# idcrook/tweeker_raytracer

Hardware: AMD Instinct MI355X
Metric: Msamples/s (paths x spp x res / s), Cornell box 1920x1080 (higher is better)
Workload: dtype f32; 1 GPU; C2: Cornell box (scene_rtigo3_cornell_box.txt: Lambert + GGX wall + mirror + glass spheres, 64,096 triangles, 8 instances), 1920x1080, 2534 spp progressive (1 spp per step), pathLengths 2 10, light 1, miss 0; launch_width=1920, batch_depth=64, parallelism=single GPU

## Files before the change

tweeker_raytracer_amd/csrc/device_api.hip:

```cpp
#include "device_types.h"
#include "bvh_build.h"
#include "error_state.h"

#include <algorithm>
#include <chrono>
#include <cmath>
#include <cstdlib>
#include <cstring>
#include <string>
#include <vector>

static thread_local std::string g_lastError;

int twkSetError(int code, const std::string& message)
{
  g_lastError = message;
  return code;
}

namespace twk {
void launchTrace(const LaunchParams& p, int depth, bool count, bool primary, int gridBlocks, hipStream_t stream);
void launchTraceQuery(const LaunchParams& p, const float* rays, unsigned int numRays, int anyHit, float* tBetaGamma, int* ids, int gridBlocks, hipStream_t stream);
void launchGenerate(const LaunchParams& p, hipStream_t stream);
void launchShade(const LaunchParams& p, int depth, bool primary, int gridBlocks, hipStream_t stream);
// ... 73 lines not shown
  bool built = false;
  bool twoLevel = true;
  int  flattenMaxTriangles = TWK_FLATTEN_TRIANGLES, flattenMaxReferences = TWK_FLATTEN_REFERENCES;
  int  maxInstanceMaterial = -1, maxInstanceLight = -1;
  TwkBuildInfo buildInfo;

  float* d_camera = nullptr;
  DevLight* d_lights = nullptr;
  DevMaterial* d_materials = nullptr; int materialCapacity = 0;
  float* d_attributes = nullptr; unsigned int* d_indices = nullptr;
  BvhNode* d_nodes = nullptr; BvhNode* d_wideNodes = nullptr ; float4* d_wideQ = nullptr; float4* d_triangles = nullptr; float4* d_shadeTriangles = nullptr; DevInstance* d_instances = nullptr;
  bool directSmallLeaves = true;  bool costedCuts = true;  bool fusedPrimary = true;  bool tileEntries = true;  bool wideRoot = true;  int wideRoot1 = 0, wideRoot2 = TWK_BVH_SENTINEL; size_t wideNodesTotal = 0;
  int4* d_tileEntries = nullptr; size_t tileEntriesCapacity = 0; TileEntriesKey tileEntriesKey = {}; uint64_t buildSerial = 0;
  float4* d_topNodes = nullptr; float4* d_topNodes7 = nullptr; bool topCache = true; int traceWavesForced = 0 ;
  float4* d_texels[3] = {nullptr, nullptr, nullptr};
  float* d_envCDF_U = nullptr; float* d_envCDF_V = nullptr;
  int tlasRoot = 0;
  size_t totalNodes = 0, totalTriangles = 0;

  int allocatedPixels = 0;
  void* d_streamBlock = nullptr;
  float4* d_outputInternal = nullptr;
  float4* d_outputExternal = nullptr; size_t outputExternalBytes = 0;
  bool outputFrame = false;
  unsigned int* d_counters = nullptr;
  unsigned long long* d_stats = nullptr;
  unsigned int* h_dropped = nullptr; unsigned int* d_dropped = nullptr;
  int* d_spill = nullptr; size_t spillLanes = 0;
  bool packedQueue = true;
  int shadeSort = 1;
  float4* d_firstHit = nullptr; int* d_firstHitInstance = nullptr;
  bool aovEnabled = false; int shaderVariant = TWK_SHADERS_RTIGO3;
  bool nextEventEstimation = true, debugExceptions = false;
  bool timeView = false; float* d_pathTime = nullptr; int timePaths = 0;
  float4* d_pathAlbedo = nullptr; float4* d_pathNormal = nullptr; int aovPaths = 0;
  float4* d_aovAlbedo = nullptr; float4* d_aovNormal = nullptr; int aovPixels = 0;
  bool captureFirstHits = false;
  bool statsEnabled = false;
  bool profileEnabled = false;
  std::vector<TimedLaunch> timed; size_t timedUsed = 0;
  float profileMs[TWK_KERNEL_COUNT] = {0, 0, 0, 0, 0};
  int   profileLaunches[TWK_KERNEL_COUNT] = {0, 0, 0, 0, 0};
  int   batchMax = 64;
  size_t streamBudgetBytes = 0;
  unsigned int pendingFirst = 0;
  int   pendingCount = 0;
  int   allocatedPaths = 0;

  hipStream_t laneStream[TWK_MAX_LANES] = {nullptr, nullptr, nullptr, nullptr};
  hipEvent_t  laneDone[TWK_MAX_LANES] = {nullptr, nullptr, nullptr, nullptr};
  hipEvent_t  laneFork = nullptr;
  int   lanesForced = 0;
  int   laneTraceWaves = 0;

  std::vector<std::vector<char>> hostScene;

  LaunchParams params;
  BvhBuilder builder;
};

static int flushPending(TwkDevice dev);

static int activate(TwkDevice dev, const char* where, bool flush = true)
{
  if (!dev) return twkSetError(TWK_ERROR_INVALID_VALUE, std::string(where) + ": NULL device handle");
  HIP_TRY(hipSetDevice(dev->ordinal));
  if (flush && dev->pendingCount > 0) return flushPending(dev);
  return TWK_SUCCESS;
}

template<typename T> static void freeDevice(T*& p) { if (p) { (void) hipFree(p); p = nullptr; } }

template<typename T> struct ScopedDeviceBuffer
{
  T* ptr = nullptr;
  ~ScopedDeviceBuffer() { if (ptr) (void) hipFree(ptr); }
  hipError_t allocate(size_t count) { return hipMalloc(&ptr, count * sizeof(T)); }
};

static void invertAffine(const float m[12], float inv[12])
{
  const double a00 = m[0], a01 = m[1], a02 = m[2],  t0 = m[3];
  const double a10 = m[4], a11 = m[5], a12 = m[6],  t1 = m[7];
  const double a20 = m[8], a21 = m[9], a22 = m[10], t2 = m[11];
  const double c00 = a11 * a22 - a12 * a21;
  const double c01 = a12 * a20 - a10 * a22;
  const double c02 = a10 * a21 - a11 * a20;
  const double det = a00 * c00 + a01 * c01 + a02 * c02;
  const double r = 1.0 / det;
  const double i00 = c00 * r, i01 = (a02 * a21 - a01 * a22) * r, i02 = (a01 * a12 - a02 * a11) * r;
  const double i10 = c01 * r, i11 = (a00 * a22 - a02 * a20) * r, i12 = (a02 * a10 - a00 * a12) * r;
  const double i20 = c02 * r, i21 = (a01 * a20 - a00 * a21) * r, i22 = (a00 * a11 - a01 * a10) * r;
  inv[0] = (float) i00; inv[1] = (float) i01; inv[2]  = (float) i02; inv[3]  = (float) -(i00 * t0 + i01 * t1 + i02 * t2);
  inv[4] = (float) i10; inv[5] = (float) i11; inv[6]  = (float) i12; inv[7]  = (float) -(i10 * t0 + i11 * t1 + i12 * t2);
  inv[8] = (float) i20; inv[9] = (float) i21; inv[10] = (float) i22; inv[11] = (float) -(i20 * t0 + i21 * t1 + i22 * t2);
}

static DevMaterial convertMaterial(const TwkMaterialGUI& g)
{
  DevMaterial m;
  memset(&m, 0, sizeof(m));
  m.textureAlbedo = g.useAlbedoTexture ? (TWK_TEXTURE_ALBEDO + 1) : 0;
  m.textureCutout = g.useCutoutTexture ? (TWK_TEXTURE_CUTOUT + 1) : 0;
  m.roughness[0] = g.roughness[0]; m.roughness[1] = g.roughness[1];
  m.indexBSDF = g.indexBSDF;
  m.albedo[0] = g.albedo[0]; m.albedo[1] = g.albedo[1]; m.albedo[2] = g.albedo[2];
// ... 18 lines not shown
}

static void refreshParams(TwkDevice dev)
{
  LaunchParams& p = dev->params;
  p.nodes = dev->d_nodes; p.wideQ = dev->d_wideQ; p.triangles = dev->d_triangles; p.shadeTriangles = dev->d_shadeTriangles; p.instances = dev->d_instances;
  p.attributes = dev->d_attributes; p.indices = dev->d_indices;
  p.materials = dev->d_materials; p.lights = dev->d_lights; p.camera = dev->d_camera;
  p.tlasRoot = dev->tlasRoot;
  p.topNodes = dev->d_topNodes; p.topNodes7 = dev->d_topNodes7;
  p.topRoot = dev->topCache ? (TWK_NODE_CACHED | 0) : dev->wideRoot1;
  p.topRoot2 = (dev->wideRoot2 == TWK_BVH_SENTINEL) ? TWK_BVH_SENTINEL : (dev->topCache ? (TWK_NODE_CACHED | 1) : dev->wideRoot2);
  p.twoLevel = dev->twoLevel ? 1 : 0;
  p.numInstances = (int) dev->instances.size();
  p.numLights = (int) dev->lights.size();
  p.numMaterials = (int) dev->materials.size();
  p.miss = dev->miss;
  p.hasCutout = 0; p.hasAlbedoTexture = 0;
  for (const DevMaterial& m : dev->materials) { if (m.textureCutout != 0) p.hasCutout = 1; if (m.textureAlbedo != 0) p.hasAlbedoTexture = 1; }
  p.traceWaves = (!dev->twoLevel && (!p.hasCutout || TWK_TRACE_CUTOUT_SEVEN) && dev->totalNodes <= (size_t) TWK_TRACE_WAVES7_MAX_NODES) ? TWK_TRACE_WAVES7 : (p.hasCutout ? (dev->twoLevel ? TWK_TRACE_WAVES_CUTOUT_OTHER : TWK_TRACE_WAVES) : TWK_TRACE_WAVES);
  if (dev->traceWavesForced == TWK_TRACE_WAVES || (dev->traceWavesForced == TWK_TRACE_WAVES7 && !dev->twoLevel)) p.traceWaves = dev->traceWavesForced;
  p.envCDF_U = dev->d_envCDF_U; p.envCDF_V = dev->d_envCDF_V;
  for (int k = 0; k < 2; ++k)
  {
    p.resolution[k]  = dev->state.resolution[k];
    p.tileSize[k]    = dev->state.tileSize[k];
    p.tileShift[k]   = calculateShift(dev->state.tileSize[k]);
    p.pathLengths[k] = dev->state.pathLengths[k];
  }
  p.deviceCount = dev->count; p.deviceIndex = dev->index; p.distribution = dev->state.distribution;
  p.launchWidth = dev->launchWidth;
  p.lensShader  = dev->state.lensShader;
  p.sceneEpsilon = dev->state.epsilonFactor * SCENE_EPSILON_SCALE;
  p.envRotation  = dev->state.envRotation;
  p.numPixels = dev->launchWidth * dev->state.resolution[1];
  p.batchCount = 1;
  p.numPaths = p.numPixels;
  p.queueStride = TWK_QUEUE_STRIDE(p.numPaths);
  p.pathBase = 0;
  p.output = dev->d_outputExternal ? dev->d_outputExternal : dev->d_outputInternal;
  p.outputFrame = (dev->d_outputExternal && dev->outputFrame) ? 1 : 0;
  p.counters = dev->d_counters;
  p.stats = dev->statsEnabled ? dev->d_stats : (dev->timeView ? dev->d_stats + TWK_STATS_WORDS / 2 : nullptr);
  p.pathTime = dev->timeView ? dev->d_pathTime : nullptr; p.clockScale = dev->state.clockFactor * 1.0e-9f;
  p.shaderVariant = dev->shaderVariant; p.shadeSort = dev->shadeSort;
  p.nextEventEstimation = dev->nextEventEstimation ? 1 : 0; p.debugExceptions = dev->debugExceptions ? 1 : 0;
  p.pathAlbedo = dev->aovEnabled ? dev->d_pathAlbedo : nullptr; p.pathNormal = dev->aovEnabled ? dev->d_pathNormal : nullptr;
  p.aovAlbedo  = dev->aovEnabled ? dev->d_aovAlbedo : nullptr;  p.aovNormal  = dev->aovEnabled ? dev->d_aovNormal : nullptr;
  p.firstHit = dev->captureFirstHits ? dev->d_firstHit : nullptr;
  p.firstHitInstance = dev->captureFirstHits ? dev->d_firstHitInstance : nullptr;
  p.traceStackSpill = dev->d_spill;
  p.droppedPushes = dev->d_dropped;
  p.packedQueue = 0;
}

static int traceGridBlocks(TwkDevice dev) { return dev->numCUs * TWK_TRACE_WAVES7; }

static int ensureStreams(TwkDevice dev, int samples = 1)
{
  const size_t wantPixels = (size_t) dev->launchWidth * (size_t) dev->state.resolution[1];
  const size_t wantPaths  = wantPixels * (size_t) (samples > 1 ? samples : 1);
  if (wantPaths >= ((size_t) 1 << 31))
    return twkSetError(TWK_ERROR_OUT_OF_MEMORY, "a pass of " + std::to_string(wantPaths) + " paths exceeds the 2^31 path indices of a wavefront pass");
  const int numPixels = (int) wantPixels;
  const int numPaths  = (int) wantPaths;
  if (numPixels > dev->allocatedPixels || dev->d_outputInternal == nullptr)
  {
    freeDevice(dev->d_outputInternal);
    freeDevice(dev->d_firstHit); freeDevice(dev->d_firstHitInstance);
    const size_t n = (size_t) numPixels;
    HIP_TRY(hipMalloc(&dev->d_outputInternal, n * sizeof(float4)));
    HIP_TRY(hipMemsetAsync(dev->d_outputInternal, 0, n * sizeof(float4), dev->stream));
    HIP_TRY(hipMalloc(&dev->d_firstHit, n * sizeof(float4)));
    HIP_TRY(hipMalloc(&dev->d_firstHitInstance, n * sizeof(int)));
    dev->allocatedPixels = numPixels;
  }
  if (numPaths > dev->allocatedPaths || dev->d_streamBlock == nullptr)
  {
    freeDevice(dev->d_streamBlock);
    const size_t n = (size_t) numPaths;
    const size_t bytes = (n + TWK_STREAM_PAD) * (15 * sizeof(float4) + 2 * sizeof(uint2) + 6 * sizeof(unsigned int)) + 4096;
    if (dev->streamBudgetBytes != 0 && n * (15 * sizeof(float4) + 2 * sizeof(uint2) + 6 * sizeof(unsigned int)) > dev->streamBudgetBytes)
      return twkSetError(TWK_ERROR_OUT_OF_MEMORY, "path streams of " + std::to_string(bytes >> 20) + " MiB exceed TWK_STREAM_BUDGET_MB");
    HIP_TRY(hipMalloc(&dev->d_streamBlock, bytes));
    dev->allocatedPaths = numPaths;
  }
  if (dev->timeView && dev->allocatedPaths > dev->timePaths)
  {
    freeDevice(dev->d_pathTime); dev->timePaths = 0;
    HIP_TRY(hipMalloc(&dev->d_pathTime, (size_t) dev->allocatedPaths * sizeof(float)));
    dev->timePaths = dev->allocatedPaths;
  }
  if (dev->aovEnabled)
  {
    if (dev->allocatedPaths > dev->aovPaths)
    {
      freeDevice(dev->d_pathAlbedo); freeDevice(dev->d_pathNormal); dev->aovPaths = 0;
      HIP_TRY(hipMalloc(&dev->d_pathAlbedo, (size_t) dev->allocatedPaths * sizeof(float4)));
      HIP_TRY(hipMalloc(&dev->d_pathNormal, (size_t) dev->allocatedPaths * sizeof(float4)));
      dev->aovPaths = dev->allocatedPaths;
    }
    if (dev->allocatedPixels > dev->aovPixels)
    {
      freeDevice(dev->d_aovAlbedo); freeDevice(dev->d_aovNormal); dev->aovPixels = 0;
      const size_t bytes = (size_t) dev->allocatedPixels * sizeof(float4);
      HIP_TRY(hipMalloc(&dev->d_aovAlbedo, bytes));
// ... 319 lines not shown
{
  if (!count) return twkSetError(TWK_ERROR_INVALID_VALUE, "twk_device_count: NULL argument");
  *count = 0;
  int n = 0;
  const hipError_t e = hipGetDeviceCount(&n);
  if (e != hipSuccess) return twkSetError(TWK_ERROR_NO_DEVICE, std::string("hipGetDeviceCount failed: ") + hipGetErrorString(e));
  *count = n;
  return TWK_SUCCESS;
}
TWK_CATCH("twk_device_count")

int twk_device_create(TwkDevice* out, int ordinal, int index, int count, int miss)
try
{
  if (!out) return twkSetError(TWK_ERROR_INVALID_VALUE, "twk_device_create: NULL out pointer");
  *out = nullptr;
  if (count < 1 || index < 0 || index >= count) return twkSetError(TWK_ERROR_INVALID_VALUE, "twk_device_create: need 0 <= index < count");
  int n = 0;
  const hipError_t e = hipGetDeviceCount(&n);
  if (e != hipSuccess || n <= 0)
    return twkSetError(TWK_ERROR_NO_DEVICE, std::string("twk_device_create: no HIP device available (") + ((e != hipSuccess) ? hipGetErrorString(e) : "device count 0") + "); this library has no CPU path");
  if (ordinal < 0 || ordinal >= n) return twkSetError(TWK_ERROR_INVALID_VALUE, "twk_device_create: device ordinal out of range");

  TwkDevice_t* dev = new TwkDevice_t();
  dev->ordinal = ordinal; dev->index = index; dev->count = count; dev->miss = miss;
  memset(&dev->params, 0, sizeof(dev->params));
  memset(&dev->state, 0, sizeof(dev->state));
  dev->state.resolution[0] = dev->state.resolution[1] = 1;
  dev->state.tileSize[0] = dev->state.tileSize[1] = 8;
  dev->state.pathLengths[0] = 2; dev->state.pathLengths[1] = 5;
  dev->state.epsilonFactor = 500.0f;
  dev->state.clockFactor = 1000.0f;

  hipError_t err = hipSetDevice(ordinal);
  if (err == hipSuccess) err = hipStreamCreateWithFlags(&dev->stream, hipStreamNonBlocking);
  hipDeviceProp_t prop;
  if (err == hipSuccess) err = hipGetDeviceProperties(&prop, ordinal);
  if (err != hipSuccess)
  {
    delete dev;
    return twkSetError(TWK_ERROR_NO_DEVICE, std::string("twk_device_create: ") + hipGetErrorString(err));
  }
  dev->numCUs = prop.multiProcessorCount > 0 ? prop.multiProcessorCount : 256;
  if (const char* e = getenv("TWK_PASS_LANES")) dev->lanesForced = std::max(0, std::min(TWK_MAX_LANES, atoi(e)));
  if (const char* e = getenv("TWK_LANE_TRACE_WAVES")) dev->laneTraceWaves = std::max(0, atoi(e));
  if (const char* e = getenv("TWK_TOP_CACHE")) dev->topCache = (atoi(e) != 0);
  if (const char* e = getenv("TWK_DIRECT_SMALL_LEAVES")) dev->directSmallLeaves = (atoi(e) != 0);
  if (const char* e = getenv("TWK_COSTED_CUTS")) dev->costedCuts = (atoi(e) != 0);
  if (const char* e = getenv("TWK_FUSED_PRIMARY")) dev->fusedPrimary = (atoi(e) != 0);
  if (const char* e = getenv("TWK_TILE_ENTRIES")) dev->tileEntries = (atoi(e) != 0);
  if (const char* e = getenv("TWK_WIDE_ROOT")) dev->wideRoot = (atoi(e) != 0);
  if (const char* e = getenv("TWK_PACKED_QUEUE")) dev->packedQueue = (atoi(e) != 0);
  if (const char* e = getenv("TWK_SHADE_SORT")) dev->shadeSort = atoi(e);
  if (const char* e = getenv("TWK_TRACE_WAVES_RUNTIME")) dev->traceWavesForced = atoi(e);
  if (const char* e = getenv("TWK_BUILD_QUALITY")) dev->builder.setQuality(atoi(e));
  memset(&dev->buildInfo, 0, sizeof(dev->buildInfo));
  if (const char* e = getenv("TWK_STREAM_BUDGET_MB")) { const long long mb = atoll(e); dev->streamBudgetBytes = (mb > 0) ? (size_t) mb << 20 : 0; }
  if (const char* e = getenv("TWK_BATCH")) { const int b = atoi(e); dev->batchMax = (b < 1) ? 1 : ((b > 64) ? 64 : b); }
  *out = dev;
  return TWK_SUCCESS;
}
TWK_CATCH("twk_device_create")

int twk_device_destroy(TwkDevice dev)
try
{
  if (!dev) return TWK_SUCCESS;
  dev->pendingCount = 0;
  (void) hipSetDevice(dev->ordinal);
  if (dev->stream) (void) hipStreamSynchronize(dev->stream);
  for (TimedLaunch& t : dev->timed) { (void) hipEventDestroy(t.start); (void) hipEventDestroy(t.stop); }
  freeDevice(dev->d_camera); freeDevice(dev->d_lights); freeDevice(dev->d_materials);
  freeDevice(dev->d_attributes); freeDevice(dev->d_indices);
  freeDevice(dev->d_nodes); freeDevice(dev->d_wideNodes); freeDevice(dev->d_wideQ); freeDevice(dev->d_triangles); freeDevice(dev->d_shadeTriangles); freeDevice(dev->d_instances);
  for (int k = 0; k < 3; ++k) freeDevice(dev->d_texels[k]);
  freeDevice(dev->d_envCDF_U); freeDevice(dev->d_envCDF_V); freeDevice(dev->d_topNodes); freeDevice(dev->d_topNodes7); freeDevice(dev->d_tileEntries);
  freeDevice(dev->d_streamBlock); freeDevice(dev->d_outputInternal);
  freeDevice(dev->d_counters); freeDevice(dev->d_stats); freeDevice(dev->d_spill); freeDevice(dev->d_pathTime);
  if (dev->h_dropped) { (void) hipHostFree(dev->h_dropped); dev->h_dropped = nullptr; dev->d_dropped = nullptr; }
  freeDevice(dev->d_firstHit); freeDevice(dev->d_firstHitInstance);
  freeDevice(dev->d_pathAlbedo); freeDevice(dev->d_pathNormal); freeDevice(dev->d_aovAlbedo); freeDevice(dev->d_aovNormal);
  dev->builder.release();
  for (int k = 1; k < TWK_MAX_LANES; ++k)
  {
    if (dev->laneStream[k]) (void) hipStreamDestroy(dev->laneStream[k]);
    if (dev->laneDone[k]) (void) hipEventDestroy(dev->laneDone[k]);
  }
  if (dev->laneFork) (void) hipEventDestroy(dev->laneFork);
  if (dev->stream) (void) hipStreamDestroy(dev->stream);
  delete dev;
  return TWK_SUCCESS;
}
TWK_CATCH("twk_device_destroy")

int twk_set_state(TwkDevice dev, const TwkDeviceState* s)
try
{
  int rc = activate(dev, "twk_set_state"); if (rc) return rc;
  if (!s) return twkSetError(TWK_ERROR_INVALID_VALUE, "twk_set_state: NULL state");
  if (s->resolution[0] < 1 || s->resolution[1] < 1) return twkSetError(TWK_ERROR_INVALID_VALUE, "twk_set_state: resolution must be >= 1");
  if (s->tileSize[0] < 1 || s->tileSize[1] < 1 || (s->tileSize[0] & (s->tileSize[0] - 1)) || (s->tileSize[1] & (s->tileSize[1] - 1)))
    return twkSetError(TWK_ERROR_INVALID_VALUE, "twk_set_state: tileSize must be a power of two");
  if (s->pathLengths[1] < 0 || s->pathLengths[1] > TWK_MAX_DEPTH) return twkSetError(TWK_ERROR_INVALID_VALUE, "twk_set_state: pathLengths.y must be in [0, 64]");
  if (s->lensShader < 0 || s->lensShader > 2) return twkSetError(TWK_ERROR_INVALID_VALUE, "twk_set_state: lensShader must be 0..2");
  HIP_TRY(hipStreamSynchronize(dev->stream));
  dev->state = *s;
// ... 966 lines not shown
```

tweeker_raytracer_amd/csrc/device_types.h:

```cpp
#pragma once
#include "device_math.h"
#include "../../include/tweeker_hip.h"

namespace twk {

static const float RT_DEFAULT_MAX      = 1.e27f;
static const float SCENE_EPSILON_SCALE = 1.0e-7f;
static const float DENOMINATOR_EPSILON = 1.0e-6f;

#define TWK_MATERIAL_STACK_EMPTY (-1)
#define TWK_MATERIAL_STACK_FIRST 0
#define TWK_MATERIAL_STACK_LAST  3
#define TWK_MATERIAL_STACK_SIZE  4
#define TWK_FLAG_HIT          0x00000001u
#define TWK_FLAG_SHADOW       0x00000002u
#define TWK_FLAG_DIFFUSE      0x00000004u
#define TWK_FLAG_LIGHT        0x00000008u
#define TWK_FLAG_FRONTFACE    0x00000010u
#define TWK_FLAG_THINWALLED   0x00000020u
#define TWK_FLAG_TRANSMISSION 0x00000100u
#define TWK_FLAG_VOLUME       0x00001000u
#define TWK_FLAG_ALBEDO       0x10000000u
#define TWK_FLAG_TERMINATE    0x80000000u
#define TWK_FLAG_CLEAR_MASK   (TWK_FLAG_DIFFUSE | TWK_FLAG_ALBEDO)
// ... 96 lines not shown
  unsigned int envWidth, envHeight;
  float envIntegral, envRotation;

  int   resolution[2];
  int   tileSize[2];
  int   tileShift[2];
  int   pathLengths[2];
  int   deviceCount, deviceIndex, distribution;
  int   launchWidth;
  int   lensShader;
  unsigned int iterationIndex;
  float sceneEpsilon;

  float4* rayOrg[2];
  float4* rayDir[2];
  unsigned int* rayPixel[2];
  float4* hitRecord;
  int*    hitInstance;
  float4* shadowOrg;
  float4* shadowDir;
  unsigned int* shadowPixel;
  float4* shadowPending;
  float4* rayThroughput[2];
  uint2*  raySeedFlags[2];
  float4* pathRadiance;
  float4* volumeStack;
  float4* pathAlbedo;
  float4* pathNormal;
  float*  pathTime;
  float   clockScale;
  float4* aovAlbedo;
  float4* aovNormal;
  int     shaderVariant;
  int     shadeSort;
  int     nextEventEstimation;
  int     debugExceptions;
  int     outputFrame;
  float4* output;
  unsigned int* counters;
  unsigned long long* stats;
  float4* firstHit;
  int*    firstHitInstance;
  int*    traceStackSpill;
  unsigned int* overflowSlots;
  int     numPixels;
  int     numPaths;
  int     batchCount;
  int     pathBase;
  const int4* tileEntries;
  int     tilesX;
  int     packedQueue;
  unsigned int queueStride;
  unsigned int* droppedPushes;
};

#ifndef TWK_QUEUE_SEGMENTS
#define TWK_QUEUE_SEGMENTS 4
#endif
#ifndef TWK_COUNTER_SEGMENT_STRIDE
#define TWK_COUNTER_SEGMENT_STRIDE 64
#endif
#define TWK_COUNTERS_PER_DEPTH (2 * TWK_QUEUE_SEGMENTS * TWK_COUNTER_SEGMENT_STRIDE + 2)
#define TWK_COUNTER_CLOSEST  0
#define TWK_COUNTER_SHADOW   (TWK_QUEUE_SEGMENTS * TWK_COUNTER_SEGMENT_STRIDE)
#define TWK_COUNTER_TICKET   (2 * TWK_QUEUE_SEGMENTS * TWK_COUNTER_SEGMENT_STRIDE)
#define TWK_COUNTER_OVERFLOW (2 * TWK_QUEUE_SEGMENTS * TWK_COUNTER_SEGMENT_STRIDE + 1)
#define TWK_QUEUE_STRIDE(numPaths) ((((unsigned int) (numPaths) / TWK_QUEUE_SEGMENTS + 255u) & ~255u) + 512u)

struct QueueSegments { unsigned int first[TWK_QUEUE_SEGMENTS]; unsigned int total; };

TWK_HD QueueSegments queueSegments(const unsigned int* counts)
{
  QueueSegments s; unsigned int sum = 0u;
  for (int k = 0; k < TWK_QUEUE_SEGMENTS; ++k) { s.first[k] = sum; sum += counts[k * TWK_COUNTER_SEGMENT_STRIDE]; }
  s.total = sum;
  return s;
}
TWK_HD QueueSegments noSegments() { QueueSegments s; for (int k = 0; k < TWK_QUEUE_SEGMENTS; ++k) s.first[k] = 0u; s.total = 0u; return s; }
TWK_HD unsigned int physicalSlot(const QueueSegments& s, unsigned int stride, unsigned int v)
{
  unsigned int k = 0u, f = 0u;
  for (int j = 1; j < TWK_QUEUE_SEGMENTS; ++j) { const bool in = v >= s.first[j]; k += in ? 1u : 0u; f = in ? s.first[j] : f; }
  return k * stride + (v - f);
}
#define TWK_MAX_DEPTH 64

#ifndef TWK_TRACE_STACK_LDS
#define TWK_TRACE_STACK_LDS   20
#endif
#ifndef TWK_TRACE_WAVES
#define TWK_TRACE_WAVES 6
#endif
#ifndef TWK_TRACE_CUTOUT_SEVEN
#define TWK_TRACE_CUTOUT_SEVEN 1
#endif
#ifndef TWK_TRACE_WAVES_CUTOUT_OTHER
#define TWK_TRACE_WAVES_CUTOUT_OTHER 5
#endif
#ifndef TWK_TRACE_WAVES_PRIMARY
#define TWK_TRACE_WAVES_PRIMARY TWK_TRACE_WAVES
#endif
#ifndef TWK_TRACE_WAVES_PRIMARY_TWO_LEVEL
#define TWK_TRACE_WAVES_PRIMARY_TWO_LEVEL 5
#endif
#define TWK_TRACE_WAVES7      7
#define TWK_TRACE_STACK_LDS7  19
#define TWK_TOP_NODES7        32
#ifndef TWK_TRACE_WAVES7_MAX_NODES
#define TWK_TRACE_WAVES7_MAX_NODES 1000000
#endif
#ifndef TWK_ENTRY_TILE
#define TWK_ENTRY_TILE 8
#endif
#define TWK_ENTRY_REFS 7
#ifndef TWK_PRIMARY_SIX
#define TWK_PRIMARY_SIX 1
#endif
#define TWK_TRACE_STACK_SPILL 72
#define TWK_TRACE_BLOCK       256
#define TWK_SHADE_BLOCKS_PER_CU 128
#ifndef TWK_SHADE_BLOCK
#define TWK_SHADE_BLOCK       256
#endif
#ifndef TWK_LANES2_MAX_PATHS
#define TWK_LANES2_MAX_PATHS 21000000
#endif
#ifndef TWK_TRACE_SMALL_CHUNK
#define TWK_TRACE_SMALL_CHUNK 64
#endif
#ifndef TWK_TRACE_CHUNK
#define TWK_TRACE_CHUNK       512
#endif

}
```

tweeker_raytracer_amd/csrc/trace_persistent.h:

```cpp
#pragma once
#include "trace_device.h"
#include "shade_device.h"

namespace twk {

TWK_D bool cutoutIgnoresCandidate(const LaunchParams& p, const TraceResult& res, bool isShadow, int q, unsigned int record, bool primary = false)
{
  const DevInstance& inst = p.instances[res.instance];
  const DevMaterial& material = p.materials[inst.material];
  if (material.textureCutout == 0) return false;
  const float4* sv = p.shadeTriangles + TWK_SHADE_RECORD * (size_t) res.triangleSlot;
  const float4 s5 = sv[5], s6 = sv[6], s7 = sv[7];
  const float alpha = 1.0f - res.beta - res.gamma;
  const V3 texcoord = v3(s5.y, s5.z, s5.w) * alpha + v3(s6.x, s6.y, s6.z) * res.beta + v3(s6.w, s7.x, s7.y) * res.gamma;
  const float opacity = intensity(v3(tex2D(p.textures[1], texcoord.x, texcoord.y)));
  if (!(opacity < 1.0f)) return false;
  float draw;
  if (isShadow)
  {
    float4 pend = p.shadowPending[record];
    unsigned int seed = __float_as_uint(pend.w);
    draw = rng(seed);
    pend.w = __uint_as_float(seed);
    p.shadowPending[record] = pend;
  }
  else
  {
    uint2 sf = p.raySeedFlags[q][record];
    draw = rng(sf.x);
    p.raySeedFlags[q][record] = sf;
  }
  if (!(opacity <= draw)) return false;
  if (isShadow) p.shadowOrg[record].w = res.t; else if (!primary) p.rayOrg[q][record].w = res.t;
  return true;
}

#ifndef TWK_TRACE_REFILL
#define TWK_TRACE_REFILL 52
#endif
#ifndef TWK_TRACE_REFILL_PRIMARY
#define TWK_TRACE_REFILL_PRIMARY 32
#endif
#ifndef TWK_TRACE_TAIL_DEN
#define TWK_TRACE_TAIL_DEN 2
#endif
#ifndef TWK_TRACE_TAIL_MIN
#define TWK_TRACE_TAIL_MIN 2u
#endif
#ifndef TWK_TRACE_NODE_NUM
#define TWK_TRACE_NODE_NUM 1
#endif
#ifndef TWK_TRACE_NODE_DEN
#define TWK_TRACE_NODE_DEN 2
#endif

template<bool COUNT, bool CUTOUT, bool TWO_LEVEL, bool W7, bool PRIMARY>
__global__ void __launch_bounds__(TWK_TRACE_BLOCK, W7 ? TWK_TRACE_WAVES7 : (CUTOUT ? ((PRIMARY || TWO_LEVEL) ? TWK_TRACE_WAVES_CUTOUT_OTHER : TWK_TRACE_WAVES) : ((PRIMARY && TWO_LEVEL) ? TWK_TRACE_WAVES_PRIMARY_TWO_LEVEL : (PRIMARY ? TWK_TRACE_WAVES_PRIMARY : TWK_TRACE_WAVES))))
traceKernel(LaunchParams p, int depth)
{
  constexpr int STACK_LDS = W7 ? TWK_TRACE_STACK_LDS7 : TWK_TRACE_STACK_LDS;
  constexpr int TOP_NODES = W7 ? TWK_TOP_NODES7 : TWK_TOP_NODES;
  constexpr int STACK_ROWS = STACK_LDS + 1;
  __shared__ int stackStorage[STACK_ROWS * TWK_TRACE_BLOCK];
  __shared__ float4 topCache[TOP_NODES * TWK_TOP_STRIDE];
  int* ldsStack = stackStorage + threadIdx.x;
  const int stride = TWK_TRACE_BLOCK;
  {
    const float4* topSource = W7 ? p.topNodes7 : p.topNodes;
    for (int i = threadIdx.x; i < TOP_NODES * 4; i += TWK_TRACE_BLOCK) topCache[(i >> 2) * TWK_TOP_STRIDE + (i & 3)] = topSource[i];
  }
  __syncthreads();

  const QueueSegments closestSegments = queueSegments(&p.counters[depth * TWK_COUNTERS_PER_DEPTH + TWK_COUNTER_CLOSEST]);
  const QueueSegments shadowSegments  = (depth > 0) ? queueSegments(&p.counters[(depth - 1) * TWK_COUNTERS_PER_DEPTH + TWK_COUNTER_SHADOW]) : noSegments();
  const unsigned int numClosest = closestSegments.total, numShadow = shadowSegments.total;
  const unsigned int total = numClosest + numShadow;
#define TWK_RECORD(slot_) (((slot_) < numClosest) ? (PRIMARY ? (slot_) : physicalSlot(closestSegments, p.queueStride, (slot_))) : physicalSlot(shadowSegments, p.queueStride, (slot_) - numClosest))

  const int q = depth & 1;
  const bool packed = !CUTOUT && !PRIMARY && p.packedQueue != 0 && depth > 0;
  const unsigned int lane = threadIdx.x & 63u;
  const unsigned long long laneBelow = (1ull << lane) - 1ull;

  unsigned int nodeCount = 0, triCount = 0, instCount = 0, closestCount = 0, shadowCount = 0, maxSteps = 0, cachedCount = 0;
  unsigned int nodeWaveSteps = 0, triWaveSteps = 0, leafWaveSteps = 0;
#define TWK_WAVE_STEP(counter) if (COUNT) { if (lane == (unsigned int) (__ffsll((long long) __ballot(true)) - 1)) ++(counter); }
  unsigned long long phaseCycles[5] = {0ull, 0ull, 0ull, 0ull, 0ull};
  unsigned long long phaseMark = COUNT ? __builtin_readcyclecounter() : 0ull;
  const unsigned long long kernelStart = phaseMark;
#define TWK_PHASE_END(k) if (COUNT) { const unsigned long long now_ = __builtin_readcyclecounter(); phaseCycles[k] += now_ - phaseMark; phaseMark = now_; }

  const unsigned int numWaves = gridDim.x * (TWK_TRACE_BLOCK / 64);
  const unsigned int waveId   = blockIdx.x * (TWK_TRACE_BLOCK / 64) + (threadIdx.x >> 6);
  unsigned int ticketSize = TWK_TRACE_CHUNK;
  const bool longQueue = total >= numWaves * ticketSize * TWK_TRACE_TAIL_MIN;
#if TWK_TRACE_SMALL_CHUNK
  if (!longQueue) ticketSize = TWK_TRACE_SMALL_CHUNK;
#else
  if (total < numWaves * ticketSize) ticketSize = min((unsigned int) TWK_TRACE_CHUNK, max(16u, ((total + numWaves - 1u) / numWaves + 15u) & ~15u));
#endif
  unsigned int nextChunk = waveId * ticketSize;
  if (nextChunk >= total) return;
  unsigned int poolBase = 0u, poolCount = 0u;
#if TWK_TRACE_TAIL_DEN
  unsigned int* ticket = &p.counters[depth * TWK_COUNTERS_PER_DEPTH + TWK_COUNTER_TICKET];
  const unsigned int staticEnd = longQueue ? ((total - total / TWK_TRACE_TAIL_DEN) / (numWaves * ticketSize)) * (numWaves * ticketSize) : total;
#else
  const unsigned int staticEnd = total;
#endif
  bool exhausted = false;

  enum : unsigned int
  {
    ST_HAS_RAY    = 1u,
    ST_ANY_HIT    = 2u,
    ST_DONE       = 4u,
    ST_SHADOW     = 8u,
    ST_RETRACE    = 16u,
    ST_OVERFLOWED = 32u,
    ST_CLOCKED    = 64u
  };
  unsigned int state = 0u;
  unsigned int slot = 0;
  V3 org = v3(0.0f), dir = v3(0.0f);
  float tmin = 0.0f;
  TraceResult res; res.t = 0.0f; res.beta = 0.0f; res.gamma = 0.0f; res.instance = -1; res.primitive = -1; res.triangleSlot = -1;
  TraceRay ray; ray.o = v3(0.0f); ray.d = v3(0.0f); ray.id = v3(0.0f);
  WoopConstants woop; woop.perm = 0u; woop.Sx = 0.0f; woop.Sy = 0.0f; woop.Sz = 0.0f;
  int currentInstance = -1, sp = 0, node = TWK_BVH_SENTINEL;
  unsigned int guard = 0;
  unsigned int rayClock = 0;

  for (;;)
  {
    if (state & ST_DONE)
    {
      const unsigned int rayCycles = COUNT ? ((state & ST_CLOCKED) ? rayClock : (unsigned int) __builtin_readcyclecounter() - rayClock) : 0u;
      state &= ~(ST_DONE | ST_CLOCKED);
      const bool isShadow = (state & ST_SHADOW) != 0u;
      if (state & ST_RETRACE)
      {
        state = (state & ~ST_RETRACE) | ST_OVERFLOWED;
        const unsigned int k = atomicAdd(&p.counters[depth * TWK_COUNTERS_PER_DEPTH + TWK_COUNTER_OVERFLOW], 1u);
        p.overflowSlots[k] = slot;
        if (PRIMARY && CUTOUT) p.hitRecord[slot] = make_float4(tmin, 0.0f, 0.0f, 0.0f);
      }
      if (COUNT) maxSteps = max(maxSteps, guard);
      const bool ignoredCandidate = CUTOUT && !(state & ST_OVERFLOWED) && res.instance >= 0 &&
                                    cutoutIgnoresCandidate(p, res, isShadow, q, TWK_RECORD(slot), PRIMARY);
      if (ignoredCandidate)
      {
        tmin = res.t;
        float4 o, d;
        if (PRIMARY)
        {
          const PrimaryRay pr = primaryRay(p, slot);
          o = make_float4(pr.origin.x, pr.origin.y, pr.origin.z, 0.0f);
          d = make_float4(pr.direction.x, pr.direction.y, pr.direction.z, RT_DEFAULT_MAX);
        }
        else
        {
          const unsigned int record = TWK_RECORD(slot);
          o = isShadow ? p.shadowOrg[record] : p.rayOrg[q][record];
          d = isShadow ? p.shadowDir[record] : p.rayDir[q][record];
        }
        org = v3(o); dir = v3(d);
        res.t = d.w; res.beta = 0.0f; res.gamma = 0.0f; res.instance = -1; res.primitive = -1; res.triangleSlot = -1;
        setupRay(ray, org, dir);
        woopSetup(dir, woop);
        if (COUNT) rayClock = (unsigned int) __builtin_readcyclecounter() - rayCycles;
        currentInstance = -1; sp = 0; node = p.topRoot; guard = 0;
        if (p.topRoot2 != TWK_BVH_SENTINEL) { ldsStack[0] = p.topRoot2; sp = 1; }
        state |= ST_HAS_RAY;
      }
      else if (state & ST_OVERFLOWED) { state &= ~ST_OVERFLOWED; }
      else if (!isShadow)
      {
        p.hitRecord[slot]   = make_float4(res.t, res.beta, res.gamma, __int_as_float(res.triangleSlot));
        p.hitInstance[slot] = res.instance;
        if (COUNT) ++closestCount;
        if (COUNT && p.pathTime != nullptr) atomicAdd(&p.pathTime[PRIMARY ? slot : (packed ? (__float_as_uint(p.rayOrg[q][TWK_RECORD(slot)].w) & TWK_PACKED_PIXEL_MASK) : p.rayPixel[q][TWK_RECORD(slot)])], float(rayCycles));
        if (p.firstHit != nullptr && depth == 0)
        {
          const unsigned int pixel = PRIMARY ? slot : p.rayPixel[q][TWK_RECORD(slot)];
          p.firstHit[pixel] = make_float4(res.t, res.beta, res.gamma, __int_as_float(res.primitive));
          p.firstHitInstance[pixel] = res.instance;
        }
      }
// ... 41 lines not shown
            slot = poolBase + rank;
            float4 o, d;
            int4 entryA = make_int4(0, 0, 0, 0), entryB = make_int4(0, 0, 0, 0);
            if (PRIMARY)
            {
              const PrimaryRay pr = primaryRay(p, slot);
              o = make_float4(pr.origin.x, pr.origin.y, pr.origin.z, p.sceneEpsilon);
              d = make_float4(pr.direction.x, pr.direction.y, pr.direction.z, pr.active ? RT_DEFAULT_MAX : -1.0f);
              state = ST_HAS_RAY;
              if (CUTOUT) p.raySeedFlags[0][slot] = make_uint2(pr.seed, 0u);
              if (p.tileEntries != nullptr)
              {
                const unsigned int launchIndex = (slot + (unsigned int) p.pathBase) % (unsigned int) p.numPixels;
                const unsigned int lx = launchIndex % (unsigned int) p.launchWidth, ly = launchIndex / (unsigned int) p.launchWidth;
                const int4* tile = p.tileEntries + 2 * ((size_t) (ly / TWK_ENTRY_TILE) * (unsigned int) p.tilesX + lx / TWK_ENTRY_TILE);
                entryA = tile[0]; entryB = tile[1];
              }
            }
            else if (slot < numClosest)
            {
              const unsigned int record = physicalSlot(closestSegments, p.queueStride, slot);
              o = p.rayOrg[q][record]; d = p.rayDir[q][record]; state = ST_HAS_RAY;
              if (packed) { o.w = p.sceneEpsilon; d.w = RT_DEFAULT_MAX; }
            }
            else
            {
              const unsigned int record = physicalSlot(shadowSegments, p.queueStride, slot - numClosest);
              o = p.shadowOrg[record]; d = p.shadowDir[record]; state = ST_HAS_RAY | ST_SHADOW | (CUTOUT ? 0u : ST_ANY_HIT);
            }
            org = v3(o); dir = v3(d); tmin = o.w;
            res.t = d.w; res.beta = 0.0f; res.gamma = 0.0f; res.instance = -1; res.primitive = -1; res.triangleSlot = -1;
            setupRay(ray, org, dir);
            woopSetup(dir, woop);
            currentInstance = -1; sp = 0; guard = 0;
            node = p.topRoot;
            if (p.topRoot2 != TWK_BVH_SENTINEL) { ldsStack[0] = p.topRoot2; sp = 1; }
            if (COUNT) rayClock = (unsigned int) __builtin_readcyclecounter();
            if (PRIMARY && entryA.x > 0)
            {
              sp = 0;
              node = entryA.y;
              const int count = entryA.x;
              if (count > 6) { ldsStack[sp * stride] = entryB.w; ++sp; }
              if (count > 5) { ldsStack[sp * stride] = entryB.z; ++sp; }
              if (count > 4) { ldsStack[sp * stride] = entryB.y; ++sp; }
              if (count > 3) { ldsStack[sp * stride] = entryB.x; ++sp; }
              if (count > 2) { ldsStack[sp * stride] = entryA.w; ++sp; }
              if (count > 1) { ldsStack[sp * stride] = entryA.z; ++sp; }
            }
          }
          poolBase += take; poolCount -= take;
        }
      }
      if (__ballot((state & ST_HAS_RAY) != 0u) == 0ull)
      {
        if (exhausted) break;
        continue;
      }
    }
    TWK_PHASE_END(0)
    for (;;)
    {
      const int roundActive = __popcll(__ballot((state & ST_HAS_RAY) != 0u));
      while ((unsigned int) node < (unsigned int) TWK_BVH_SENTINEL)
      {
        {
          float4 n0, n1, n2, n3;
          if (node & TWK_NODE_CACHED)
          {
            const float4* w = topCache + (node & 0xff) * TWK_TOP_STRIDE;
            if (COUNT) ++cachedCount;
            n0 = w[0]; n1 = w[1]; n2 = w[2]; n3 = w[3];
          }
          else
          {
            const float4* w = p.wideQ + 4 * (size_t) node;
            n0 = w[0]; n1 = w[1]; n2 = w[2]; n3 = w[3];
          }
          ++guard;
          if (COUNT) ++nodeCount;
          TWK_WAVE_STEP(nodeWaveSteps)
          int r0 = __float_as_int(n3.x), r1 = __float_as_int(n3.y), r2 = __float_as_int(n3.z), r3 = __float_as_int(n3.w);
          asm volatile("" : "+v"(r0), "+v"(r1), "+v"(r2), "+v"(r3));
          const float ax = n0.w * ray.id.x, ay = n1.x * ray.id.y, az = n1.y * ray.id.z;
          const float bx = __builtin_fmaf(n0.x, ray.id.x, -ray.ood.x), by = __builtin_fmaf(n0.y, ray.id.y, -ray.ood.y), bz = __builtin_fmaf(n0.z, ray.id.z, -ray.ood.z);
          const bool negX = ray.id.x < 0.0f, negY = ray.id.y < 0.0f, negZ = ray.id.z < 0.0f;
          const unsigned int qlx = __float_as_uint(n1.z), qly = __float_as_uint(n1.w), qlz = __float_as_uint(n2.x);
          const unsigned int qhx = __float_as_uint(n2.y), qhy = __float_as_uint(n2.z), qhz = __float_as_uint(n2.w);
          const unsigned int qnx = negX ? qhx : qlx, qfx = negX ? qlx : qhx;
          const unsigned int qny = negY ? qhy : qly, qfy = negY ? qly : qhy;
          const unsigned int qnz = negZ ? qhz : qlz, qfz = negZ ? qlz : qhz;
          float t0, t1, t2, t3;
  #define TWK_Q(word, k) ((float) (((word) >> (8 * (k))) & 0xffu))
  #define TWK_SLAB(k, tk) slabTestGrid(ax, ay, az, bx, by, bz, TWK_Q(qnx, k), TWK_Q(qny, k), TWK_Q(qnz, k), TWK_Q(qfx, k), TWK_Q(qfy, k), TWK_Q(qfz, k), tmin, res.t, tk)
          const bool h0 = TWK_SLAB(0, t0);
          const bool h1 = TWK_SLAB(1, t1);
          const bool h2 = TWK_SLAB(2, t2);
          const bool h3 = TWK_SLAB(3, t3);
  #undef TWK_SLAB
  #undef TWK_Q
          const float inf = __uint_as_float(0x7f800000u);
          t0 = h0 ? t0 : inf; t1 = h1 ? t1 : inf; t2 = h2 ? t2 : inf; t3 = h3 ? t3 : inf;
  #define TWK_CE(ta, ra, tb, rb) { const bool sw = (tb) < (ta); const float tl = sw ? (tb) : (ta); (tb) = sw ? (ta) : (tb); (ta) = tl; const int rl = sw ? (rb) : (ra); (rb) = sw ? (ra) : (rb); (ra) = rl; }
          TWK_CE(t0, r0, t1, r1) TWK_CE(t2, r2, t3, r3) TWK_CE(t0, r0, t2, r2) TWK_CE(t1, r1, t3, r3) TWK_CE(t1, r1, t2, r2)
  #undef TWK_CE
          const int hits = (int) h0 + (int) h1 + (int) h2 + (int) h3;
// ... 26 lines not shown
        TWK_WAVE_STEP(leafWaveSteps)
        if (TWO_LEVEL && node == TWK_BVH_SENTINEL)
        {
          sp -= 4;
          woop.perm = (unsigned int) ldsStack[sp * stride];
          woop.Sx = __int_as_float(ldsStack[(sp + 1) * stride]);
          woop.Sy = __int_as_float(ldsStack[(sp + 2) * stride]);
          woop.Sz = __int_as_float(ldsStack[(sp + 3) * stride]);
          setupRay(ray, org, dir);
          currentInstance = -1;
          pop = 1u;
        }
        else
        {
          const int payload = ~node;
          if (TWO_LEVEL && currentInstance < 0 && !(payload & TWK_LEAF_WORLD))
          {
            const float4* rec = reinterpret_cast<const float4*>(p.instances + payload);
            const float4 r0 = rec[0], r1 = rec[1], r2 = rec[2], r3 = rec[3];
            if (COUNT) ++instCount;
            if (sp + 5 > STACK_LDS) state = (state & ~ST_HAS_RAY) | ST_DONE | ST_RETRACE;
            else
            {
              ldsStack[sp * stride] = (int) woop.perm;
              ldsStack[(sp + 1) * stride] = __float_as_int(woop.Sx);
              ldsStack[(sp + 2) * stride] = __float_as_int(woop.Sy);
              ldsStack[(sp + 3) * stride] = __float_as_int(woop.Sz);
              ldsStack[(sp + 4) * stride] = TWK_BVH_SENTINEL;
              sp += 5;
              float m[12];
              m[0] = r0.x; m[1] = r0.y; m[2] = r0.z; m[3] = r0.w;
              m[4] = r1.x; m[5] = r1.y; m[6] = r1.z; m[7] = r1.w;
              m[8] = r2.x; m[9] = r2.y; m[10] = r2.z; m[11] = r2.w;
              const V3 objOrg = transformPoint(m, org);
              const V3 objDir = transformVector(m, dir);
              woopSetup(objDir, woop);
              setupRay(ray, objOrg, objDir);
              currentInstance = payload;
              node = __float_as_int(r3.x);
            }
          }
          else
          {
            triFirst = payload & 0x0fffffff; triLast = triFirst + ((payload >> 28) & 3);
            pop = 1u;
          }
        }

      }

      TWK_PHASE_END(2)
#define TWK_MERGE_HIT(hit_, t_, beta_, gamma_, inst_, prim_, ts_)                                                              \
      {                                                                                                                        \
        const bool closer = (hit_) & (((t_) < res.t) |                                                                         \
                                      (((t_) == res.t) & (res.instance >= 0) &                                                 \
                                       (((inst_) < res.instance) | (((inst_) == res.instance) & ((prim_) < res.primitive))))); \
        res.t = closer ? (t_) : res.t; res.beta = closer ? (beta_) : res.beta; res.gamma = closer ? (gamma_) : res.gamma;      \
        res.instance = closer ? (inst_) : res.instance; res.primitive = closer ? (prim_) : res.primitive;                      \
        res.triangleSlot = closer ? (ts_) : res.triangleSlot;                                                                  \
        if (closer & ((state & ST_ANY_HIT) != 0u))                                                                             \
        {                                                                                                                      \
          pop = 0u; state = (state & ~ST_HAS_RAY) | ST_DONE; triLast = -1;                                                     \
        }                                                                                                                      \
      }
      for (int ts = triFirst; ts <= triLast; ++ts)
      {
        const float4* tri = p.triangles + 3 * (size_t) ts;
        const float4 a = tri[0], b = tri[1], c = tri[2];
        if (COUNT) ++triCount;
        TWK_WAVE_STEP(triWaveSteps)
        float t, beta, gamma;
        const bool hit = woopIntersect(woop, ray.o, v3(a), v3(b), v3(c), tmin, t, beta, gamma);
        const int prim = __float_as_int(a.w);
        const int triInstance = (TWO_LEVEL && currentInstance >= 0) ? currentInstance : __float_as_int(b.w);
        TWK_MERGE_HIT(hit, t, beta, gamma, triInstance, prim, ts)
      }
#undef TWK_MERGE_HIT
      TWK_PHASE_END(3)

      if (pop)
      {
        if (sp == 0) state = (state & ~ST_HAS_RAY) | ST_DONE;
        else { --sp; node = ldsStack[sp * stride]; }
      }
      if (COUNT) { if ((state & (ST_DONE | ST_CLOCKED)) == ST_DONE) { rayClock = (unsigned int) __builtin_readcyclecounter() - rayClock; state |= ST_CLOCKED; } }
      TWK_PHASE_END(4)
      if (!(state & ST_HAS_RAY)) node = TWK_BVH_SENTINEL;
      const unsigned long long active = __ballot((state & ST_HAS_RAY) != 0u);
      if (active == 0ull) break;
      if (!exhausted && __popcll(active) < min(PRIMARY ? TWK_TRACE_REFILL_PRIMARY : TWK_TRACE_REFILL, (int) ticketSize)) break;
    }
  }

  if (COUNT)
  {
    const unsigned long long kernelEnd = __builtin_readcyclecounter();
    atomicAdd(&p.stats[0], (unsigned long long) closestCount);
    atomicAdd(&p.stats[1], (unsigned long long) shadowCount);
    atomicAdd(&p.stats[2], (unsigned long long) nodeCount);
    atomicAdd(&p.stats[3], (unsigned long long) triCount);
    atomicAdd(&p.stats[4], (unsigned long long) instCount);
    atomicMax(&p.stats[7], (unsigned long long) maxSteps);
    if (nodeWaveSteps) atomicAdd(&p.stats[13], (unsigned long long) nodeWaveSteps);
    if (triWaveSteps)  atomicAdd(&p.stats[14], (unsigned long long) triWaveSteps);
    if (leafWaveSteps) atomicAdd(&p.stats[15], (unsigned long long) leafWaveSteps);
    if (cachedCount)   atomicAdd(&p.stats[16], (unsigned long long) cachedCount);
    if (lane == 0)
    {
      for (int k = 0; k < 5; ++k) atomicAdd(&p.stats[18 + k], phaseCycles[k]);
      atomicAdd(&p.stats[23], kernelEnd - kernelStart);
    }
  }
#undef TWK_WAVE_STEP
#undef TWK_PHASE_END
#undef TWK_RECORD
}

}
```

Before: 3444 Msamples/s.

## Split straggler rays across idle lanes by stealing BVH stack entries in trace tail

Once the ray queue is exhausted and a wave has fewer than traceSplit active lanes, idle lanes take the bottom BVH stack entry from a lane that is still traversing and trace that subtree as helpers. Helper results are merged back into the parent lane with the closest-hit tie-break rules, and any-hit or retrace termination is propagated. The aim is to cut the long rundown where a few lanes keep the whole wave busy. The cost is extra shuffles, ballots and state bookkeeping in the traversal loop, more register pressure, and harder-to-verify correctness for any-hit and retrace cases.

```diff
diff --git a/tweeker_raytracer_amd/csrc/device_api.hip b/tweeker_raytracer_amd/csrc/device_api.hip
--- a/tweeker_raytracer_amd/csrc/device_api.hip
+++ b/tweeker_raytracer_amd/csrc/device_api.hip
@@ -149,6 +149,7 @@
   hipEvent_t  laneFork = nullptr;
   int   lanesForced = 0;
   int   laneTraceWaves = 0;
+  int   traceSplit = TWK_TRACE_SPLIT_DEFAULT;
 
   std::vector<std::vector<char>> hostScene;
 
@@ -273,6 +274,7 @@
   p.traceStackSpill = dev->d_spill;
   p.droppedPushes = dev->d_dropped;
   p.packedQueue = 0;
+  p.traceSplit = dev->traceSplit;
 }
 
 static int traceGridBlocks(TwkDevice dev) { return dev->numCUs * TWK_TRACE_WAVES7; }
@@ -698,6 +700,7 @@
   if (const char* e = getenv("TWK_WIDE_ROOT")) dev->wideRoot = (atoi(e) != 0);
   if (const char* e = getenv("TWK_PACKED_QUEUE")) dev->packedQueue = (atoi(e) != 0);
   if (const char* e = getenv("TWK_SHADE_SORT")) dev->shadeSort = atoi(e);
+  if (const char* e = getenv("TWK_TRACE_SPLIT")) dev->traceSplit = std::max(0, std::min(64, atoi(e)));
   if (const char* e = getenv("TWK_TRACE_WAVES_RUNTIME")) dev->traceWavesForced = atoi(e);
   if (const char* e = getenv("TWK_BUILD_QUALITY")) dev->builder.setQuality(atoi(e));
   memset(&dev->buildInfo, 0, sizeof(dev->buildInfo));
diff --git a/tweeker_raytracer_amd/csrc/device_types.h b/tweeker_raytracer_amd/csrc/device_types.h
--- a/tweeker_raytracer_amd/csrc/device_types.h
+++ b/tweeker_raytracer_amd/csrc/device_types.h
@@ -172,6 +172,7 @@
   int     packedQueue;
   unsigned int queueStride;
   unsigned int* droppedPushes;
+  int     traceSplit;
 };
 
 #ifndef TWK_QUEUE_SEGMENTS
@@ -245,6 +246,9 @@
 #ifndef TWK_LANES2_MAX_PATHS
 #define TWK_LANES2_MAX_PATHS 21000000
 #endif
+#ifndef TWK_TRACE_SPLIT_DEFAULT
+#define TWK_TRACE_SPLIT_DEFAULT 8
+#endif
 #ifndef TWK_TRACE_SMALL_CHUNK
 #define TWK_TRACE_SMALL_CHUNK 64
 #endif
diff --git a/tweeker_raytracer_amd/csrc/trace_persistent.h b/tweeker_raytracer_amd/csrc/trace_persistent.h
--- a/tweeker_raytracer_amd/csrc/trace_persistent.h
+++ b/tweeker_raytracer_amd/csrc/trace_persistent.h
@@ -35,6 +35,22 @@
   return true;
 }
 
+TWK_D bool hitPrecedes(bool hit, float t, int inst, int prim, const TraceResult& res)
+{
+  return hit & ((t < res.t) | ((t == res.t) & (res.instance >= 0) & ((inst < res.instance) | ((inst == res.instance) & (prim < res.primitive)))));
+}
+
+TWK_D unsigned int nthSetBit(unsigned long long m, unsigned int n)
+{
+  unsigned int pos = 0u;
+  for (int w = 32; w > 0; w >>= 1)
+  {
+    const unsigned int below = (unsigned int) __popcll(m & ((1ull << w) - 1ull));
+    if (n >= below) { n -= below; m >>= w; pos += w; }
+  }
+  return pos;
+}
+
 #ifndef TWK_TRACE_REFILL
 #define TWK_TRACE_REFILL 52
 #endif
@@ -61,6 +77,8 @@
   constexpr int STACK_LDS = W7 ? TWK_TRACE_STACK_LDS7 : TWK_TRACE_STACK_LDS;
   constexpr int TOP_NODES = W7 ? TWK_TOP_NODES7 : TWK_TOP_NODES;
   constexpr int STACK_ROWS = STACK_LDS + 1;
+  constexpr bool SPLIT = !COUNT && !CUTOUT && !TWO_LEVEL && !(W7 && PRIMARY && TWK_PRIMARY_SIX);
+  const int splitLanes = SPLIT ? p.traceSplit : 0;
   __shared__ int stackStorage[STACK_ROWS * TWK_TRACE_BLOCK];
   __shared__ float4 topCache[TOP_NODES * TWK_TOP_STRIDE];
   int* ldsStack = stackStorage + threadIdx.x;
@@ -88,7 +106,15 @@
   unsigned long long phaseCycles[5] = {0ull, 0ull, 0ull, 0ull, 0ull};
   unsigned long long phaseMark = COUNT ? __builtin_readcyclecounter() : 0ull;
   const unsigned long long kernelStart = phaseMark;
+#ifndef TWK_TRACE_RUNDOWN
+#define TWK_TRACE_RUNDOWN 0
+#endif
+#if TWK_TRACE_RUNDOWN
+#define TWK_PHASE_END(k) if (COUNT) { const unsigned long long now_ = __builtin_readcyclecounter(); const int a_ = __popcll(__ballot((state & ST_HAS_RAY) != 0u)); \
+                                      phaseCycles[!exhausted ? 0 : (a_ <= 1 ? 1 : (a_ <= 4 ? 2 : (a_ <= 16 ? 3 : 4)))] += now_ - phaseMark; phaseMark = now_; }
+#else
 #define TWK_PHASE_END(k) if (COUNT) { const unsigned long long now_ = __builtin_readcyclecounter(); phaseCycles[k] += now_ - phaseMark; phaseMark = now_; }
+#endif
 
   const unsigned int numWaves = gridDim.x * (TWK_TRACE_BLOCK / 64);
   const unsigned int waveId   = blockIdx.x * (TWK_TRACE_BLOCK / 64) + (threadIdx.x >> 6);
@@ -118,7 +144,11 @@
     ST_SHADOW     = 8u,
     ST_RETRACE    = 16u,
     ST_OVERFLOWED = 32u,
-    ST_CLOCKED    = 64u
+    ST_CLOCKED    = 64u,
+    ST_HELPER     = 128u,
+    ST_PARENT_SHIFT = 8u,
+    ST_CHILD      = 1u << 16,
+    ST_CHILDREN   = 0x7fu << 16
   };
   unsigned int state = 0u;
   unsigned int slot = 0;
@@ -133,7 +163,39 @@
 
   for (;;)
   {
-    if (state & ST_DONE)
+    if (splitLanes > 0 && exhausted && __ballot((state & ST_HELPER) != 0u) != 0ull)
+    {
+      const bool helping = (state & (ST_HELPER | ST_HAS_RAY)) == (ST_HELPER | ST_HAS_RAY);
+      const int parent = helping ? (int) ((state >> ST_PARENT_SHIFT) & 63u) : (int) lane;
+      const unsigned int parentState = (unsigned int) __shfl((int) state, parent);
+      const float pt = __shfl(res.t, parent);
+      const int pi = __shfl(res.instance, parent), pp = __shfl(res.primitive, parent);
+      const bool adopt = helping && hitPrecedes(pi >= 0, pt, pi, pp, res);
+      const int from = adopt ? parent : (int) lane;
+      res.t = adopt ? pt : res.t; res.instance = adopt ? pi : res.instance; res.primitive = adopt ? pp : res.primitive;
+      res.beta = __shfl(res.beta, from); res.gamma = __shfl(res.gamma, from); res.triangleSlot = __shfl(res.triangleSlot, from);
+      if (helping && (((state & ST_ANY_HIT) && res.instance >= 0) || (parentState & ST_RETRACE))) { state = (state & ~ST_HAS_RAY) | ST_DONE; node = TWK_BVH_SENTINEL; }
+      for (;;)
+      {
+        const unsigned long long ready = __ballot((state & (ST_HELPER | ST_DONE | ST_CHILDREN)) == (ST_HELPER | ST_DONE));
+        if (ready == 0ull) break;
+        const int h = __ffsll((long long) ready) - 1;
+        const unsigned int hs = (unsigned int) __builtin_amdgcn_readlane((int) state, h);
+        const float ht = __int_as_float(__builtin_amdgcn_readlane(__float_as_int(res.t), h));
+        const float hb = __int_as_float(__builtin_amdgcn_readlane(__float_as_int(res.beta), h));
+        const float hg = __int_as_float(__builtin_amdgcn_readlane(__float_as_int(res.gamma), h));
+        const int hi = __builtin_amdgcn_readlane(res.instance, h), hp = __builtin_amdgcn_readlane(res.primitive, h), hts = __builtin_amdgcn_readlane(res.triangleSlot, h);
+        if (lane == ((hs >> ST_PARENT_SHIFT) & 63u))
+        {
+          if (hitPrecedes(hi >= 0, ht, hi, hp, res)) { res.t = ht; res.beta = hb; res.gamma = hg; res.instance = hi; res.primitive = hp; res.triangleSlot = hts; }
+          state = (state - ST_CHILD) | (hs & ST_RETRACE);
+          if ((state & ST_HAS_RAY) && (((state & ST_ANY_HIT) && res.instance >= 0) || (state & ST_RETRACE))) { state = (state & ~ST_HAS_RAY) | ST_DONE; node = TWK_BVH_SENTINEL; }
+        }
+        if (lane == (unsigned int) h) { state = 0u; node = TWK_BVH_SENTINEL; }
+      }
+    }
+
+    if (SPLIT ? ((state & (ST_DONE | ST_HELPER | ST_CHILDREN)) == ST_DONE) : ((state & ST_DONE) != 0u))
     {
       const unsigned int rayCycles = COUNT ? ((state & ST_CLOCKED) ? rayClock : (unsigned int) __builtin_readcyclecounter() - rayClock) : 0u;
       state &= ~(ST_DONE | ST_CLOCKED);
@@ -281,6 +343,39 @@
           poolBase += take; poolCount -= take;
         }
       }
+      if (splitLanes > 0 && exhausted)
+      {
+        const unsigned long long running = __ballot((state & ST_HAS_RAY) != 0u);
+        const unsigned long long freeLanes = __ballot((state & (ST_HAS_RAY | ST_DONE | ST_CHILDREN)) == 0u);
+        const unsigned long long donors = __ballot((state & ST_HAS_RAY) && sp > 0);
+        const unsigned int pairs = min((unsigned int) __popcll(freeLanes), (unsigned int) __popcll(donors));
+        if (__popcll(running) < splitLanes && pairs != 0u)
+        {
+          const bool isFree = (freeLanes >> lane) & 1ull;
+          const unsigned int freeRank = (unsigned int) __popcll(freeLanes & laneBelow);
+          const bool thief = isFree && freeRank < pairs;
+          const int victim = thief ? (int) nthSetBit(donors, freeRank) : (int) lane;
+          slot = (unsigned int) __shfl((int) slot, victim);
+          ray.o.x = __shfl(ray.o.x, victim); ray.o.y = __shfl(ray.o.y, victim); ray.o.z = __shfl(ray.o.z, victim);
+          ray.id.x = __shfl(ray.id.x, victim); ray.id.y = __shfl(ray.id.y, victim); ray.id.z = __shfl(ray.id.z, victim);
+          ray.ood.x = __shfl(ray.ood.x, victim); ray.ood.y = __shfl(ray.ood.y, victim); ray.ood.z = __shfl(ray.ood.z, victim);
+          woop.perm = (unsigned int) __shfl((int) woop.perm, victim);
+          woop.Sx = __shfl(woop.Sx, victim); woop.Sy = __shfl(woop.Sy, victim); woop.Sz = __shfl(woop.Sz, victim);
+          tmin = __shfl(tmin, victim);
+          res.t = __shfl(res.t, victim); res.beta = __shfl(res.beta, victim); res.gamma = __shfl(res.gamma, victim);
+          res.instance = __shfl(res.instance, victim); res.primitive = __shfl(res.primitive, victim); res.triangleSlot = __shfl(res.triangleSlot, victim);
+          if (thief) { node = ldsStack[victim - (int) lane]; sp = 0; guard = 0; }
+          if (((donors >> lane) & 1ull) && (unsigned int) __popcll(donors & laneBelow) < pairs)
+          {
+#pragma unroll 1
+            for (int i = 1; i < sp; ++i) ldsStack[(i - 1) * stride] = ldsStack[i * stride];
+            --sp;
+            state += ST_CHILD;
+          }
+          const unsigned int vState = (unsigned int) __shfl((int) state, victim);
+          if (thief) state = ST_HAS_RAY | ST_HELPER | (vState & (ST_ANY_HIT | ST_SHADOW)) | ((unsigned int) victim << ST_PARENT_SHIFT);
+        }
+      }
       if (__ballot((state & ST_HAS_RAY) != 0u) == 0ull)
       {
         if (exhausted) break;
@@ -413,9 +508,7 @@
       TWK_PHASE_END(2)
 #define TWK_MERGE_HIT(hit_, t_, beta_, gamma_, inst_, prim_, ts_)                                                              \
       {                                                                                                                        \
-        const bool closer = (hit_) & (((t_) < res.t) |                                                                         \
-                                      (((t_) == res.t) & (res.instance >= 0) &                                                 \
-                                       (((inst_) < res.instance) | (((inst_) == res.instance) & ((prim_) < res.primitive))))); \
+        const bool closer = hitPrecedes((hit_), (t_), (inst_), (prim_), res);                                                  \
         res.t = closer ? (t_) : res.t; res.beta = closer ? (beta_) : res.beta; res.gamma = closer ? (gamma_) : res.gamma;      \
         res.instance = closer ? (inst_) : res.instance; res.primitive = closer ? (prim_) : res.primitive;                      \
         res.triangleSlot = closer ? (ts_) : res.triangleSlot;                                                                  \
@@ -450,6 +543,8 @@
       const unsigned long long active = __ballot((state & ST_HAS_RAY) != 0u);
       if (active == 0ull) break;
       if (!exhausted && __popcll(active) < min(PRIMARY ? TWK_TRACE_REFILL_PRIMARY : TWK_TRACE_REFILL, (int) ticketSize)) break;
+      if (splitLanes > 0 && exhausted && __popcll(active) < splitLanes &&
+          __ballot((state & (ST_HAS_RAY | ST_CHILDREN)) == 0u) != 0ull && __ballot((state & ST_HAS_RAY) && sp > 0) != 0ull) break;
     }
   }
 
```

Result: no change. 3443 Msamples/s (median of 4 runs) (-0.0%).
